# scroll-tech/zkvm-prover

Measured on AMD Instinct MI355X. Metric: chunk STARK proofs/sec (2^22-row trace), higher is better.
Workload: dtype u32; 1 GPU; full STARK proof: 2^22 x 300 degree-3 AIR + 2^22 x 2 Fibonacci AIR, blow-up 2, 100 queries, PoW 16+16 (SURVEY.md 8(d) cfg #4); proof_bytes=1128348, resident_key_bytes_per_pipeline=13503716096, inflight_per_gpu=3, parallelism=3 independent proof(s) in flight per GPU (one HIP stream each)

## Files before the change

include/zkhip.h:

```cpp
#ifndef ZKHIP_H
#define ZKHIP_H
#include <stddef.h>
#include <stdint.h>

#ifdef __cplusplus
extern "C" {
#endif

#define ZKHIP_OK 0
#define ZKHIP_ERR_NO_DEVICE (-1)
#define ZKHIP_ERR_HIP (-2)
#define ZKHIP_ERR_INVALID (-3)
#define ZKHIP_ERR_NOMEM (-4)
#define ZKHIP_ERR_SMALL_BUFFER (-5)
#define ZKHIP_ERR_POW_FAILED (-6)
#define ZKHIP_ERR_VERIFY (-7)
#define ZKHIP_ERR_CONSTRAINT (-8)

#define ZKHIP_DIGEST_WORDS 8

typedef struct zkhip_ctx zkhip_ctx;

uint32_t zkhip_version(void);

// ... 541 lines not shown
int zkhip_recursion_witness(zkhip_recursion *r, const uint8_t *const *proofs, const size_t *proof_lens, const uint32_t *const *const *child_pvs,
                            size_t n_present, uint32_t *node_pvs_out);
int zkhip_recursion_witness_uniform(zkhip_recursion *r, const uint8_t *const *proofs, const size_t *proof_lens, const uint32_t *const *const *child_pvs,
                                    const uint32_t *child_prep_commits, const int *child_is_leaf, const uint32_t leaf_commit[8],
                                    const uint32_t internal_commit[8], size_t n_present, uint32_t *node_pvs_out);
int zkhip_recursion_witness_deferral(zkhip_recursion *r, const uint8_t *const *proofs, const size_t *proof_lens, const uint32_t *const *const *child_pvs,
                                     const uint32_t *child_aux, const uint32_t acc_start[8], size_t n_present, uint32_t *node_pvs_out);
size_t zkhip_recursion_n_aux(const zkhip_recursion *r);
int zkhip_recursion_wires(const zkhip_recursion *r, uint32_t *out, size_t cap_words, size_t *n_words);
int zkhip_recursion_tracegen(zkhip_ctx *ctx, zkhip_recursion *r, uint32_t *d_gate_trace, uint32_t *d_p2_trace, uint32_t *d_pv_trace);

typedef struct {
    int host_sponge;
    uint32_t host_sponge_min_words;
    int jit;
    uint32_t jit_min_log_work;
    char jit_cache_dir[256];
    int quot_slices;
    uint32_t grind_sweep_shift;
    uint32_t coop_max_log, coop_inj_max_log;
    uint32_t top_max_log;
    uint32_t commit_parts, side_cus;
    uint32_t witness_threads;
    int pin_witness, parallel_queries;
    int self_check;
    int tree_store_early;
    uint32_t hash_block;
    int coop_fused;
    int rows_in_bulk;
    uint32_t rows_coop_max_log;
    uint32_t ntt_log_lanes;
    uint32_t quot_streams;
    uint32_t ntt_pass_form;
} zkhip_config;
int zkhip_tables_canonical(zkhip_ctx *ctx, int on);
int zkhip_jit_prewarm(const zkhip_air *airs, size_t n_airs, unsigned log_blowup, const char *cache_dir, size_t *n_ok);
void zkhip_config_default(zkhip_config *out);
unsigned zkhip_host_cpus(void);
int zkhip_ctx_get_config(zkhip_ctx *ctx, zkhip_config *out);
int zkhip_has_test_kernels(void);
int zkhip_ctx_set_config(zkhip_ctx *ctx, const zkhip_config *cfg);
int zkhip_set_process_config(const zkhip_config *cfg);

int zkhip_profile_enable(zkhip_ctx *ctx, int on);
typedef struct {
    char name[48];
    uint64_t launches;
    double total_ms;
} zkhip_kernel_stat;
int zkhip_profile_read(zkhip_ctx *ctx, zkhip_kernel_stat *out, size_t cap);
int zkhip_profile_reset(zkhip_ctx *ctx);

#ifdef __cplusplus
}
#endif
#endif
```

integration/hip-backend/src/ffi.rs:

```rust
#![allow(non_camel_case_types)]
use std::os::raw::{c_char, c_double, c_int, c_uint, c_void};

pub const ZKHIP_OK: c_int = 0;
pub const ZKHIP_ERR_NO_DEVICE: c_int = -1;
pub const ZKHIP_ERR_HIP: c_int = -2;
pub const ZKHIP_ERR_INVALID: c_int = -3;
pub const ZKHIP_ERR_NOMEM: c_int = -4;
pub const ZKHIP_ERR_SMALL_BUFFER: c_int = -5;
pub const ZKHIP_ERR_POW_FAILED: c_int = -6;
pub const ZKHIP_ERR_VERIFY: c_int = -7;
pub const ZKHIP_ERR_CONSTRAINT: c_int = -8;
pub const ZKHIP_DIGEST_WORDS: usize = 8;
pub const ZKHIP_KECCAK_F_WIDTH: usize = 2633;
pub const ZKHIP_INT256_ALU_WIDTH: usize = 101;
pub const ZKHIP_INT256_MUL_WIDTH: usize = 161;
pub const ZKHIP_MODMUL_WIDTH: usize = 325;
pub const ZKHIP_EC_WIDTH: usize = 772;
pub const ZKHIP_FP2_WIDTH: usize = 648;
pub const ZKHIP_FP2_RECORD_WORDS: usize = 33;
pub const ZKHIP_INT256_CMP_WIDTH: usize = 103;
pub const ZKHIP_INT256_SHIFT_WIDTH: usize = 189;
pub const ZKHIP_EC_RECORD_WORDS: usize = 41;
pub const ZKHIP_GKR_MAX_LOG_N: c_uint = 28;
pub const ZKHIP_WHIR_MAX_ROUNDS: usize = 32;
// ... 173 lines not shown
    pub min_log_height: [c_uint; 2],
    pub n_leaf_shapes: usize,
    pub app_id: *const u32,
    pub region_index: u32,
}

#[repr(C)]
#[derive(Clone, Copy)]
pub struct zkhip_config {
    pub host_sponge: c_int,
    pub host_sponge_min_words: u32,
    pub jit: c_int,
    pub jit_min_log_work: u32,
    pub jit_cache_dir: [c_char; 256],
    pub quot_slices: c_int,
    pub grind_sweep_shift: u32,
    pub coop_max_log: u32,
    pub coop_inj_max_log: u32,
    pub top_max_log: u32,
    pub commit_parts: u32,
    pub side_cus: u32,
    pub witness_threads: u32,
    pub pin_witness: c_int,
    pub parallel_queries: c_int,
    pub self_check: c_int,
    pub tree_store_early: c_int,
    pub hash_block: u32,
    pub coop_fused: c_int,
    pub rows_in_bulk: c_int,
    pub rows_coop_max_log: u32,
    pub ntt_log_lanes: u32,
    pub quot_streams: u32,
    pub ntt_pass_form: u32,
}

#[repr(C)]
#[derive(Clone, Copy)]
pub struct zkhip_kernel_stat {
    pub name: [c_char; 48],
    pub launches: u64,
    pub total_ms: c_double,
}

extern "C" {
    pub fn zkhip_version() -> u32;

    pub fn zkhip_ctx_create(device: c_int, out: *mut *mut zkhip_ctx) -> c_int;
    pub fn zkhip_ctx_destroy(ctx: *mut zkhip_ctx);
    pub fn zkhip_last_error(ctx: *const zkhip_ctx) -> *const c_char;
    pub fn zkhip_set_stream(ctx: *mut zkhip_ctx, hip_stream: *mut c_void) -> c_int;
    pub fn zkhip_sync(ctx: *mut zkhip_ctx) -> c_int;
    pub fn zkhip_set_commit_pipeline(ctx: *mut zkhip_ctx, parts: c_uint) -> c_int;
    pub fn zkhip_set_cu_partition(ctx: *mut zkhip_ctx, side_cus: c_uint) -> c_int;

    pub fn zkhip_malloc(ctx: *mut zkhip_ctx, bytes: usize, dptr: *mut *mut c_void) -> c_int;
    pub fn zkhip_free(ctx: *mut zkhip_ctx, dptr: *mut c_void) -> c_int;
    pub fn zkhip_h2d(ctx: *mut zkhip_ctx, dst: *mut c_void, src: *const c_void, bytes: usize) -> c_int;
    pub fn zkhip_d2h(ctx: *mut zkhip_ctx, dst: *mut c_void, src: *const c_void, bytes: usize) -> c_int;
    pub fn zkhip_host_alloc(ctx: *mut zkhip_ctx, bytes: usize, hptr: *mut *mut c_void) -> c_int;
    pub fn zkhip_host_free(ctx: *mut zkhip_ctx, hptr: *mut c_void) -> c_int;
    pub fn zkhip_h2d_async(ctx: *mut zkhip_ctx, dst: *mut c_void, src_pinned: *const c_void, bytes: usize) -> c_int;
    pub fn zkhip_zero(ctx: *mut zkhip_ctx, dptr: *mut c_void, bytes: usize) -> c_int;
    pub fn zkhip_to_monty(ctx: *mut zkhip_ctx, d: *mut u32, n: usize) -> c_int;
    pub fn zkhip_from_monty(ctx: *mut zkhip_ctx, d: *mut u32, n: usize) -> c_int;

    pub fn zkhip_ntt_batch(ctx: *mut zkhip_ctx, d_mat: *mut u32, log_n: c_uint, width: usize, stride: usize,
// ... 381 lines not shown
```

zkvm-prover_amd/_binding.py:

```python
import ctypes as C
import os
import re

import numpy as np

P = 2013265921
_HERE = os.path.dirname(os.path.abspath(__file__))
_ROOT = os.path.dirname(_HERE)
_LIB = None


class ZkhipError(RuntimeError):
    pass


def library_path():
    return os.path.join(_HERE, "libzkhip.so")


def declared_symbols():
    with open(os.path.join(_ROOT, "include", "zkhip.h")) as f:
        txt = f.read()
    txt = re.sub(r"/\*.*?\*/", "", txt, flags=re.S)
    return sorted(set(re.findall(r"\b(zkhip_[a-z0-9_]+)\s*\(", txt)))
# ... 24 lines not shown
        return p


class _Air(C.Structure):
    _fields_ = [("program", C.POINTER(C.c_uint32)), ("program_len", C.c_size_t), ("log_height", C.c_uint),
                ("width", C.c_size_t), ("n_pvs", C.c_size_t), ("prep_trace", C.POINTER(C.c_uint32)),
                ("prep_commit", C.POINTER(C.c_uint32))]


class _ProofLayout(C.Structure):
    _fields_ = [(n, C.c_size_t) for n in ("n_words", "root_main", "roots_cached", "n_cached", "root_perm", "exposed", "n_exposed", "root_quot", "opened",
                                          "n_opened", "fri_layers", "n_fri_layers", "final_poly", "n_final_poly", "query_pow", "queries",
                                          "query_words", "n_queries")]


class _V1Summary(C.Structure):
    _fields_ = [(n, C.c_size_t) for n in ("n_proofs", "n_airs", "n_queries", "n_fri_layers", "n_final_poly", "n_main_commits",
                                          "n_after_challenge_commits", "n_preprocessed", "n_input_batches")] + \
               [("log_max_height", C.c_uint), ("log_blowup", C.c_uint), ("has_logup_pow", C.c_int), ("log_degree", C.c_uint * 64)]


class _RecursionStmt(C.Structure):
    _fields_ = [("n_state", C.c_size_t), ("start_air", C.POINTER(C.c_uint32)), ("start_idx", C.POINTER(C.c_uint32)),
                ("end_air", C.POINTER(C.c_uint32)), ("end_idx", C.POINTER(C.c_uint32)), ("child_is_node", C.c_int),
                ("uniform", C.c_int), ("min_log_height", C.c_uint * 2), ("n_leaf_shapes", C.c_size_t), ("app_id", C.POINTER(C.c_uint32)),
                ("region_index", C.c_uint32)]


class Config(C.Structure):
    _fields_ = [("host_sponge", C.c_int), ("host_sponge_min_words", C.c_uint32), ("jit", C.c_int), ("jit_min_log_work", C.c_uint32),
                ("jit_cache_dir", C.c_char * 256), ("quot_slices", C.c_int), ("grind_sweep_shift", C.c_uint32), ("coop_max_log", C.c_uint32),
                ("coop_inj_max_log", C.c_uint32), ("top_max_log", C.c_uint32), ("commit_parts", C.c_uint32), ("side_cus", C.c_uint32), ("witness_threads", C.c_uint32),
                ("pin_witness", C.c_int), ("parallel_queries", C.c_int), ("self_check", C.c_int), ("tree_store_early", C.c_int), ("hash_block", C.c_uint32), ("coop_fused", C.c_int),
                ("rows_in_bulk", C.c_int), ("rows_coop_max_log", C.c_uint32), ("ntt_log_lanes", C.c_uint32), ("quot_streams", C.c_uint32), ("ntt_pass_form", C.c_uint32)]

    @classmethod
    def default(cls):
        c = cls()
        load_library().zkhip_config_default(C.byref(c))
        return c


class _KernelStat(C.Structure):
    _fields_ = [("name", C.c_char * 48), ("launches", C.c_uint64), ("total_ms", C.c_double)]


def load_library():
    global _LIB
    if _LIB is not None:
        return _LIB
    path = library_path()
    if not os.path.exists(path):
        raise ZkhipError("libzkhip.so not built: run `python -c 'import __graft_entry__ as g; g.build()'` "
                         "(or make -C zkvm-prover_amd/csrc)")
    import torch

    lib = C.CDLL(path)
    vp, sz, u32p, uip = C.c_void_p, C.c_size_t, C.POINTER(C.c_uint32), C.POINTER(C.c_uint)
    sig = {
        "zkhip_version": (C.c_uint32, []),
        "zkhip_ctx_create": (C.c_int, [C.c_int, C.POINTER(vp)]),
        "zkhip_ctx_destroy": (None, [vp]),
        "zkhip_last_error": (C.c_char_p, [vp]),
        "zkhip_set_stream": (C.c_int, [vp, vp]),
        "zkhip_sync": (C.c_int, [vp]),
        "zkhip_set_commit_pipeline": (C.c_int, [vp, C.c_uint]),
        "zkhip_set_cu_partition": (C.c_int, [vp, C.c_uint]),
# ... 2017 lines not shown
```

zkvm-prover_amd/csrc/api.hip:

```cpp
#include <sched.h>
#include <cstring>
#include <thread>
#include <dlfcn.h>
#include <sys/stat.h>
#include <mutex>
#include <string.h>

#include <algorithm>
#include <mutex>
#include <unordered_map>

#include "transcript.hpp"
#include "zkhip_internal.hpp"

namespace zk {

int set_error(zkhip_ctx* ctx, int code, const std::string& msg) {
    if (ctx) ctx->last_error = msg;
    return code;
}

int get_scratch(zkhip_ctx* ctx, int slot, size_t bytes, void** out) {
    if (bytes == 0) bytes = 16;
    if (ctx->scratch_bytes[slot] < bytes) {
// ... 163 lines not shown
    }();
    return cached;
}

void zkhip_config_default(zkhip_config* c) {
    if (!c) return;
    auto num = [](const char* name, uint32_t dflt, uint32_t lo = 0, uint32_t hi = 0xffffffffu) {
        if (!getenv(name)) return dflt;
        const long long v = atoll(getenv(name));
        return (uint32_t)std::min<long long>(hi, std::max<long long>(lo, v));
    };
    memset(c, 0, sizeof *c);
    c->host_sponge = getenv("ZKHIP_NO_HOST_SPONGE") ? 0 : 1;
    c->host_sponge_min_words = num("ZKHIP_HOST_SPONGE_MIN_WORDS", 8192u);
    c->jit = getenv("ZKHIP_NO_JIT") ? 0 : getenv("ZKHIP_FORCE_JIT") ? 2 : 1;
    c->jit_min_log_work = num("ZKHIP_JIT_MIN_LOG_WORK", 26u, 0, 62);
    c->quot_slices = getenv("ZKHIP_NO_QUOT_SLICES") ? 0 : 1;
    c->grind_sweep_shift = num("ZKHIP_GRIND_SWEEP_SHIFT", 0u, 0, 8);
    c->coop_max_log = num("ZKHIP_COOP_MAX_LOG", 15u, 0, 27), c->coop_inj_max_log = num("ZKHIP_COOP_INJ_MAX_LOG", 15u, 0, 27);
    c->top_max_log = num("ZKHIP_TOP_MAX_LOG", 6u, 0, 8);
    c->commit_parts = num("ZKHIP_COMMIT_PARTS", 0u, 0, 8), c->side_cus = num("ZKHIP_SIDE_CUS", 0u);
    c->witness_threads = num("ZKHIP_WITNESS_THREADS", 0u);
    c->pin_witness = getenv("ZKHIP_NO_PIN_WITNESS") ? 0 : 1;
    c->parallel_queries = getenv("ZKHIP_RECURSION_SERIAL_QUERIES") ? 0 : 1;
    c->self_check = getenv("ZKHIP_SELF_CHECK") ? 1 : 0;
#ifdef ZKHIP_TEST_KERNELS
    c->tree_store_early = getenv("ZKHIP_TREE_STORE_EARLY") ? 1 : 0;
#endif
    c->hash_block = num("ZKHIP_HASH_BLOCK", 256u, 64, 768) / 64 * 64;
    c->coop_fused = getenv("ZKHIP_NO_COOP_FUSED") ? 0 : 1;
    c->rows_in_bulk = getenv("ZKHIP_NO_ROWS_IN_BULK") ? 0 : 1;
    c->rows_coop_max_log = num("ZKHIP_ROWS_COOP_MAX_LOG", 15u, 0, 27);
    c->ntt_log_lanes = num("ZKHIP_NTT_LOG_LANES", 10u, 8, 10);
    c->ntt_pass_form = num("ZKHIP_NTT_PASS_FORM", 0u, 0, 2);
    c->quot_streams = num("ZKHIP_QUOT_STREAMS", 0u, 0, 4);
    std::string dir;
    if (const char* e = getenv("ZKHIP_JIT_CACHE_DIR")) {
        dir = e;
    } else {
        Dl_info info;
        if (dladdr((const void*)&zkhip_config_default, &info) && info.dli_fname) {
            std::string p = info.dli_fname;
            const size_t slash = p.rfind('/');
            p = (slash == std::string::npos ? std::string(".") : p.substr(0, slash)) + "/jit_cache";
            struct stat st;
            if (stat(p.c_str(), &st) == 0 && S_ISDIR(st.st_mode)) dir = p;
        }
    }
    if (dir.size() < sizeof c->jit_cache_dir) memcpy(c->jit_cache_dir, dir.c_str(), dir.size() + 1);
}
extern "C++" {
namespace zk {
static zkhip_config g_process_config;
static std::once_flag g_process_config_once;
static std::mutex g_process_config_mu;
zkhip_config process_config() {
    std::call_once(g_process_config_once, [] { zkhip_config_default(&g_process_config); });
    std::lock_guard<std::mutex> lk(g_process_config_mu);
    return g_process_config;
}
}
}
int zkhip_set_process_config(const zkhip_config* cfg) {
    if (!cfg) return ZKHIP_ERR_INVALID;
    (void)zk::process_config();
    std::lock_guard<std::mutex> lk(zk::g_process_config_mu);
    zk::g_process_config = *cfg;
    return ZKHIP_OK;
}
int zkhip_tables_canonical(zkhip_ctx* ctx, int on) {
    if (!ctx) return ZKHIP_ERR_INVALID;
    ctx->tables_canonical = on != 0;
    return ZKHIP_OK;
}

int zkhip_has_test_kernels(void) {
#ifdef ZKHIP_TEST_KERNELS
    return 1;
#else
    return 0;
#endif
}

int zkhip_ctx_get_config(zkhip_ctx* ctx, zkhip_config* out) {
    if (!ctx || !out) return ZKHIP_ERR_INVALID;
    *out = ctx->cfg;
    return ZKHIP_OK;
}
int zkhip_ctx_set_config(zkhip_ctx* ctx, const zkhip_config* cfg) {
    if (!ctx || !cfg) return ZKHIP_ERR_INVALID;
    if (cfg->jit < 0 || cfg->jit > 2 || cfg->coop_max_log > 27 || cfg->coop_inj_max_log > 27 || cfg->rows_coop_max_log > 27 || cfg->ntt_log_lanes < 8 || cfg->ntt_log_lanes > 10 || cfg->ntt_pass_form > 2 || cfg->quot_streams > 4 || cfg->jit_min_log_work > 62 || cfg->top_max_log > 8 || cfg->grind_sweep_shift > 8 ||
        cfg->commit_parts > 8 || cfg->side_cus >= (unsigned)ctx->cu_count || cfg->hash_block < 64 || cfg->hash_block > 768 || cfg->hash_block % 64)
        return set_error(ctx, ZKHIP_ERR_INVALID, "zkhip_ctx_set_config: field out of range (jit 0..2, coop_* <= 27, rows_coop_max_log <= 27, ntt_log_lanes 8..10, ntt_pass_form <= 2, quot_streams <= 4, jit_min_log_work <= 62, top_max_log <= 8, grind_sweep_shift <= 8, commit_parts <= 8, side_cus < CUs, hash_block a multiple of 64 in 64..768)");
#ifndef ZKHIP_TEST_KERNELS
    if (cfg->tree_store_early)
        return set_error(ctx, ZKHIP_ERR_INVALID, "zkhip_ctx_set_config: tree_store_early names TEST kernels that this library was built without (libzkhip_test.so holds them)");
#endif
    ZK_TRY(zkhip_set_cu_partition(ctx, cfg->side_cus));
    ctx->cfg = *cfg;
    ctx->cfg.jit_cache_dir[sizeof ctx->cfg.jit_cache_dir - 1] = 0;
    ctx->commit_parts = cfg->commit_parts;
    return ZKHIP_OK;
}

void zkhip_ctx_destroy(zkhip_ctx* ctx) {
    if (!ctx) return;
    (void)hipSetDevice(ctx->device);
    (void)hipStreamSynchronize(ctx->stream);
    profile_flush(ctx);
    if (ctx->d_tw_fwd) (void)hipFree(ctx->d_tw_fwd);
    if (ctx->d_tw_inv) (void)hipFree(ctx->d_tw_inv);
    for (auto& kv : ctx->lde_tables) (void)hipFree(kv.second);
    for (int i = 0; i < 8; i++)
        if (ctx->scratch[i]) (void)hipFree(ctx->scratch[i]);
    if (ctx->side_stream) (void)hipStreamDestroy(ctx->side_stream);
    if (ctx->hash_stream) (void)hipStreamDestroy(ctx->hash_stream);
    for (auto& q : ctx->quot_streams)
        if (q) (void)hipStreamDestroy(q);
    if (ctx->quot_fork) (void)hipEventDestroy(ctx->quot_fork);
    for (auto& e : ctx->quot_join)
        if (e) (void)hipEventDestroy(e);
    if (ctx->d_deferred_bad) (void)hipFree(ctx->d_deferred_bad);
    if (ctx->gkr_ws) (void)hipFree(ctx->gkr_ws);
    if (ctx->h_sponge) (void)hipHostFree(ctx->h_sponge);
    if (ctx->own_stream) (void)hipStreamDestroy(ctx->own_stream);
    for (auto& e : ctx->pipe_ev)
// ... 340 lines not shown
```

zkvm-prover_amd/csrc/ntt.hip:

```cpp
#include <stdlib.h>
#include <string.h>

#include <algorithm>

#include "lds_barrier.hpp"
#include "zkhip_internal.hpp"

namespace zk {

__global__ void k_gen_twiddles(uint32_t* fwd, uint32_t* inv, uint32_t w, uint32_t winv, size_t half) {
    size_t e = (size_t)blockIdx.x * blockDim.x + threadIdx.x;
    if (e >= half) return;
    fwd[e] = mpow(w, e);
    inv[e] = mpow(winv, e);
}

int ensure_twiddles(zkhip_ctx* ctx, unsigned log_n) {
    if (log_n < 1) log_n = 1;
    if (log_n > 27) return set_error(ctx, ZKHIP_ERR_INVALID, "transform size exceeds two-adicity 27");
    if (ctx->tw_log >= log_n) return ZKHIP_OK;
    unsigned want = std::max(log_n, 16u);
    if (ctx->d_tw_fwd) {
        ZK_HIP_CHECK(ctx, hipStreamSynchronize(ctx->stream));
        ZK_HIP_CHECK(ctx, hipFree(ctx->d_tw_fwd));
// ... 82 lines not shown
    }
    if (wide) {
        for (unsigned e = tid; e < total; e += nt) {
            unsigned r = e >> a.log_c, c = e & C_mask;
            dst[base + ((size_t)r << log_S) + c] = lds[e];
        }
    } else {
        const unsigned grp_mask = (1u << (a.log_r + log_S)) - 1u;
        for (unsigned e = tid; e < total; e += nt) {
            unsigned g = e >> (a.log_r + log_S), rem = e & grp_mask;
            unsigned r = rem >> log_S, low = rem & S_mask;
            dst[base + e] = lds[(r << a.log_c) + (g << log_S) + low];
        }
    }
}

struct Pass4Args {
    const uint32_t* src;
    uint32_t* dst;
    size_t src_col_stride, dst_col_stride;
    const uint32_t* tw;
    size_t in_x_stride, in_rs;
    size_t out_x_stride, out_hi_stride, out_lo_stride;
    unsigned log_sub, log_m, log_r, log_f, log_lo, tw_log, log_c;
    int in_tw;
    unsigned log_prev, log_tt;
    uint32_t tw_a, tw_bx;
    int br_src;
    const uint32_t* scale_col;
    const uint32_t* scale_row;
    const uint32_t* scale_rho;
    const uint32_t* const* src_cols;
    uint32_t* const* dst_cols;
};

template <int Q>
__device__ __forceinline__ void dif_unit(uint32_t (&v)[16], const uint32_t* twl, unsigned j, unsigned log_rq,
                                         unsigned tshift) {
#pragma unroll
    for (int t = 0; t < Q; t++) {
        constexpr int dummy = 0;
        (void)dummy;
        const int half = 1 << (Q - 1 - t);
#pragma unroll
        for (int kl = 0; kl < half; kl++) {
            const uint32_t w = twl[((j + ((unsigned)kl << log_rq)) << t) << tshift];
#pragma unroll
            for (int blk = 0; blk < (1 << t); blk++) {
                const int ka = blk * 2 * half + kl, kb = ka + half;
                const uint32_t x = v[ka], y = v[kb];
                v[ka] = madd(x, y);
                v[kb] = canon_signed(smml((int32_t)(x - y), (int32_t)w));
            }
        }
    }
}

template <int Q>
__device__ __forceinline__ void lds_round(uint32_t* lv, const uint32_t* twl, unsigned log_r, unsigned log_rcur,
                                          unsigned log_c, unsigned tid, unsigned nt) {
    const unsigned log_rq = log_rcur - Q;
    const unsigned n_units = 1u << (log_r - Q + log_c);
    const unsigned cmask = (1u << log_c) - 1u, pitch = (1u << log_c) + 1u;
    for (unsigned u = tid; u < n_units; u += nt) {
        const unsigned c = u & cmask, jj = u >> log_c;
        const unsigned j = jj & ((1u << log_rq) - 1u), blk = jj >> log_rq;
// ... 326 lines not shown
        t = mmul(sc, sr);
    } else {
        if constexpr (MODE == P4_IN_TW) {
            const uint32_t kc = bitrev32(F0 + c, LOG_F);
            const unsigned sh = a.tw_log - LOG_M;
            t = a.tw[(size_t)(kc * j) << sh];
            rho = a.tw[(size_t)(kc << LOG_RQ) << sh];
        }
        const global_words tile_src = uniform_global((a.src_cols ? a.src_cols[mcol] : a.src + mcol * a.src_col_stride) + ((size_t)sub << LOG_M) + F0);
        const uint32_t lane_off = (j << LOG_F) + c;
#pragma unroll
        for (int k = 0; k < 16; k++) v[k] = uniform_global(tile_src + ((size_t)k << (LOG_RQ + LOG_F)))[lane_off];
    }
#pragma unroll
    for (unsigned i = 0; i < (R >> 1) / NT; i++) twl[tid + i * NT] = twe[i];
    if constexpr (MODE != P4_PLAIN) scale_geometric(v, t, rho);
    zk_syncthreads();
    {
        uint32_t w[15];
        load_unit_twiddles<4, LOG_RQ, 0>(twl, j, w);
        dif_unit_w<4>(v, w);
        uint32_t* base = lv + j * pitch + c;
#pragma unroll
        for (int k = 0; k < 16; k++) base[(k << LOG_RQ) * pitch] = v[k];
    }
    zk_syncthreads();
    lds_rounds_ct<LOG_R, LOG_C, LOG_RQ, NT>(lv, twl, tid);
    const global_words dst = uniform_global((a.dst_cols ? a.dst_cols[mcol] : a.dst + mcol * a.dst_col_stride) + ((size_t)sub << LOG_M) + ((size_t)F0 << LOG_R));
    const uint32_t* lrow = lv + tid * pitch;
#pragma unroll
    for (unsigned i = 0; i < (R * C) / NT; i++) {
        const unsigned cc = (NT * i) >> LOG_R, p0 = (NT * i) & (R - 1u);
        uniform_global(dst + ((size_t)cc << LOG_R) + p0)[tid] = lrow[p0 * pitch + cc];
    }
}

struct LdeFusedArgs {
    const uint32_t* src;
    size_t src_col_stride;
    uint32_t* dst;
    size_t dst_col_stride;
    const uint32_t *tw_inv, *tw_fwd;
    unsigned tw_log, log_m, log_cosets;
    const uint32_t *scale_col, *scale_row, *scale_rho;
};
template <int LOG_R, int LOG_C, int MIN_WAVES>
__global__ __launch_bounds__(1024, MIN_WAVES) void k_ntt_lde_fused(LdeFusedArgs a) {
    constexpr int LOG_T = 10;
    static_assert(LOG_R - 4 + LOG_C == LOG_T, "one radix-16 unit per lane");
    constexpr unsigned NT = 1u << LOG_T;
    extern __shared__ uint32_t sm[];
    constexpr unsigned R = 1u << LOG_R, C = 1u << LOG_C, pitch = C + 1u;
    constexpr int LOG_RQ = LOG_R - 4;
    constexpr unsigned log_f = LOG_R;
    uint32_t* lv = sm;
    uint32_t* twl = sm + R * pitch;
    const unsigned tid = threadIdx.x;
    for (unsigned e = tid; e < (R >> 1); e += NT) twl[e] = a.tw_inv[(size_t)e << (a.tw_log - LOG_R)];
    const size_t mcol = blockIdx.y;
    unsigned tile = blockIdx.x;
    if (LOG_C == 3) {
        unsigned k = gridDim.x >> 3;
        if (k > 16u) k = 16u;
        if (k >= 2u && (k & (k - 1u)) == 0 && (gridDim.x & (8u * k - 1u)) == 0) {
            const unsigned within = tile & (8u * k - 1u);
            tile = (tile & ~(8u * k - 1u)) | ((within & 7u) * k) | (within >> 3);
// ... 89 lines not shown
static constexpr unsigned MAX_LOG_R = 11;
static constexpr unsigned P4_MIN_LOG_M = 12;

struct BrSrc {
    const uint32_t *scale_col, *scale_row, *scale_rho;
};
static unsigned fourstep_split(unsigned log_n, unsigned a[3]) {
    const unsigned n_pass = std::max(2u, (log_n + MAX_LOG_R - 1) / MAX_LOG_R);
    a[0] = a[1] = a[2] = 0;
    for (unsigned p = 0; p < n_pass; p++) a[p] = log_n / n_pass + (p < log_n % n_pass ? 1 : 0);
    return n_pass;
}
static int pass_scratch(zkhip_ctx* ctx, unsigned log_n, size_t words, uint32_t** t1, uint32_t** t2) {
    const bool three = log_n > 2 * MAX_LOG_R;
    void* tmp;
    ZK_TRY(get_scratch(ctx, 4, words * 4 * (three ? 2 : 1), &tmp));
    *t1 = (uint32_t*)tmp;
    *t2 = three ? *t1 + words : nullptr;
    return ZKHIP_OK;
}

typedef void (*Pass4Kernel)(Pass4Args);
struct Pass4Shape {
    unsigned log_r, log_c, log_t;
    Pass4Kernel kernel;
};
#define ZK_P4_CT(R_, C_, T_) {R_, C_, T_, k_ntt_pass4_ct<R_, C_, T_>}
static const Pass4Shape P4_SHAPES[] = {
    ZK_P4_CT(11, 3, 10), ZK_P4_CT(10, 4, 10), ZK_P4_CT(9, 5, 10), ZK_P4_CT(8, 6, 10), ZK_P4_CT(7, 7, 10),
    ZK_P4_CT(10, 3, 9),  ZK_P4_CT(9, 4, 9),   ZK_P4_CT(8, 5, 9),  ZK_P4_CT(7, 6, 9),
    ZK_P4_CT(10, 2, 8),  ZK_P4_CT(9, 3, 8),   ZK_P4_CT(8, 4, 8),  ZK_P4_CT(7, 5, 8),
};
#undef ZK_P4_CT
static const Pass4Kernel P4_SQ11[3] = {k_ntt_pass4_ct_sq<ShapeSq11, P4_PLAIN>, k_ntt_pass4_ct_sq<ShapeSq11, P4_IN_TW>,
                                       k_ntt_pass4_ct_sq<ShapeSq11, P4_BR_SRC>};
static bool pass4_is_sq11(const Pass4Args& pa, unsigned n_pass, unsigned n_x, unsigned log_n) {
    return n_pass == 2 && n_x == 1 && log_n == 22 && pa.log_r == 11 && pa.log_f == 11 && pa.log_c == 3 && pa.log_lo == 0 && pa.in_x_stride == 0 &&
           pa.out_x_stride == 0 && pa.out_hi_stride == ((size_t)1 << 11) && !(pa.br_src && pa.in_tw) &&
           (!pa.in_tw || (pa.log_prev == 11 && pa.log_tt == 22 && pa.tw_a == 1 && pa.tw_bx == 0));
}
static Pass4Kernel pass4_kernel_for(const Pass4Args& pa, unsigned log_t, int pass_form, unsigned n_pass, unsigned n_x, unsigned log_n) {
    if (pass_form == 0 && pass4_is_sq11(pa, n_pass, n_x, log_n)) return P4_SQ11[pa.br_src ? P4_BR_SRC : pa.in_tw ? P4_IN_TW : P4_PLAIN];
    for (const Pass4Shape& sh : P4_SHAPES)
        if (sh.log_r == pa.log_r && sh.log_c == pa.log_c && sh.log_t == log_t) return sh.kernel;
    return k_ntt_pass4;
}

static int ntt_dif_fourstep(zkhip_ctx* ctx, const uint32_t* src, size_t src_stride, uint32_t* dst, size_t dst_stride,
                            uint32_t* tmp, uint32_t* tmp2, size_t tmp_stride, unsigned log_n, size_t width,
                            unsigned log_sub, bool inverse, const BrSrc* brsrc = nullptr,
                            const uint32_t* const* src_cols = nullptr, uint32_t* const* dst_cols = nullptr) {
    static DeviceOnce attr_set;
    if (attr_set.need(ctx->device)) {
        const int lds_max = ((17u << MAX_LOG_R) + (1u << (MAX_LOG_R - 1))) * 4;
        for (const Pass4Shape& sh : P4_SHAPES) ZK_HIP_CHECK(ctx, hipFuncSetAttribute((const void*)sh.kernel, hipFuncAttributeMaxDynamicSharedMemorySize, lds_max));
        for (Pass4Kernel k : P4_SQ11) ZK_HIP_CHECK(ctx, hipFuncSetAttribute((const void*)k, hipFuncAttributeMaxDynamicSharedMemorySize, lds_max));
        ZK_HIP_CHECK(ctx, hipFuncSetAttribute((const void*)k_ntt_pass4, hipFuncAttributeMaxDynamicSharedMemorySize, lds_max));
        attr_set.mark(ctx->device);
    }
    unsigned a[3];
    const unsigned n_pass = fourstep_split(log_n, a);
    const uint32_t* tw = inverse ? ctx->d_tw_inv : ctx->d_tw_fwd;
    auto launch = [&](Pass4Args& pa, const uint32_t* s, size_t ss, uint32_t* d, size_t ds, unsigned n_x) -> int {
        pa.src = s;
        pa.src_col_stride = ss;
        pa.dst = d;
        pa.dst_col_stride = ds;
        pa.tw = tw;
        pa.tw_log = ctx->tw_log;
        pa.log_sub = log_sub;
        pa.log_m = log_n;
        const unsigned R = 1u << pa.log_r;
        pa.log_c = pa.log_r >= 11 ? 3u : (pa.log_r >= 7 ? 14u - pa.log_r : 4u);
        unsigned log_t = 10;
        if (pa.log_r >= 7 && pa.log_r <= 10 && ctx->cfg.ntt_log_lanes >= 8 && ctx->cfg.ntt_log_lanes <= 9) {
            const unsigned lc = ctx->cfg.ntt_log_lanes + 4 - pa.log_r;
            if (lc >= 2 && lc <= pa.log_f) log_t = ctx->cfg.ntt_log_lanes, pa.log_c = lc;
        }
        if (pa.log_c > pa.log_f) pa.log_c = pa.log_f;
        const unsigned C = 1u << pa.log_c;
        const unsigned threads = std::min(1024u, std::max(64u, (R >> 4) * C));
        const size_t lds = ((size_t)R * (C + 1) + (R >> 1)) * 4;
        dim3 grid(n_x << (pa.log_f - pa.log_c), (unsigned)(width << log_sub));
        KernelScope ks(ctx, inverse ? "ntt_pass_inv" : "ntt_pass_fwd");
        hipLaunchKernelGGL(pass4_kernel_for(pa, log_t, ctx->cfg.ntt_pass_form, n_pass, n_x, log_n), grid, dim3(threads), lds, ctx->stream, pa);
        ZK_HIP_CHECK(ctx, hipGetLastError());
        return ZKHIP_OK;
    };
    Pass4Args pa;
    memset(&pa, 0, sizeof pa);
    auto first_pass_src = [&]() {
        if (brsrc) {
            pa.br_src = 1;
            pa.scale_col = brsrc->scale_col, pa.scale_row = brsrc->scale_row, pa.scale_rho = brsrc->scale_rho;
        }
    };
    if (n_pass == 2) {
        const unsigned a1 = a[0], a2 = a[1];
        pa.log_r = a1, pa.log_f = a2, pa.in_x_stride = 0, pa.in_rs = (size_t)1 << a2;
        pa.out_x_stride = 0, pa.out_hi_stride = (size_t)1 << a1, pa.out_lo_stride = 0, pa.log_lo = 0, pa.in_tw = 0;
        first_pass_src();
        pa.src_cols = src_cols;
        ZK_TRY(launch(pa, src, src_stride, tmp, tmp_stride, 1));
        pa.src_cols = nullptr, pa.dst_cols = nullptr;
        pa.br_src = 0;
        pa.log_r = a2, pa.log_f = a1, pa.in_rs = (size_t)1 << a1, pa.out_hi_stride = (size_t)1 << a2;
        pa.in_tw = 1, pa.log_prev = a1, pa.log_tt = log_n, pa.tw_a = 1, pa.tw_bx = 0;
        pa.dst_cols = dst_cols;
        ZK_TRY(launch(pa, tmp, tmp_stride, dst, dst_stride, 1));
        pa.src_cols = nullptr, pa.dst_cols = nullptr;
    } else {
        const unsigned a1 = a[0], a2 = a[1], a3 = a[2];
        pa.log_r = a1, pa.log_f = a2 + a3, pa.in_x_stride = 0, pa.in_rs = (size_t)1 << (a2 + a3);
        pa.out_x_stride = 0, pa.log_lo = a3, pa.out_lo_stride = (size_t)1 << (a1 + a2), pa.out_hi_stride = (size_t)1 << a1;
        pa.in_tw = 0;
        first_pass_src();
        pa.src_cols = src_cols;
        ZK_TRY(launch(pa, src, src_stride, tmp, tmp_stride, 1));
// ... 459 lines not shown
```

Before: 13.83 proofs/s.

## Process runs of columns per block in square 2^11 NTT pass, prefetching next column

Adds a variant of the square 2^11x2^11 four-step NTT pass kernel in which each block handles a run of consecutive matrix columns (default 4). Twiddles are loaded into LDS once per block, and the global load of the next column is issued before the current column's results are written out, overlapping load latency with the LDS butterfly rounds and the stores. The variant becomes the default (pass_form 0), and the old kernel stays reachable as pass_form 3. In exchange the grid gets fewer blocks, which may reduce occupancy and tail balance, and register pressure rises from the prefetched values.

```diff
diff --git a/include/zkhip.h b/include/zkhip.h
--- a/include/zkhip.h
+++ b/include/zkhip.h
@@ -597,6 +597,7 @@
     uint32_t ntt_log_lanes;
     uint32_t quot_streams;
     uint32_t ntt_pass_form;
+    uint32_t ntt_col_run;
 } zkhip_config;
 int zkhip_tables_canonical(zkhip_ctx *ctx, int on);
 int zkhip_jit_prewarm(const zkhip_air *airs, size_t n_airs, unsigned log_blowup, const char *cache_dir, size_t *n_ok);
diff --git a/integration/hip-backend/src/ffi.rs b/integration/hip-backend/src/ffi.rs
--- a/integration/hip-backend/src/ffi.rs
+++ b/integration/hip-backend/src/ffi.rs
@@ -229,6 +229,7 @@
     pub ntt_log_lanes: u32,
     pub quot_streams: u32,
     pub ntt_pass_form: u32,
+    pub ntt_col_run: u32,
 }
 
 #[repr(C)]
diff --git a/zkvm-prover_amd/_binding.py b/zkvm-prover_amd/_binding.py
--- a/zkvm-prover_amd/_binding.py
+++ b/zkvm-prover_amd/_binding.py
@@ -80,7 +80,8 @@
                 ("jit_cache_dir", C.c_char * 256), ("quot_slices", C.c_int), ("grind_sweep_shift", C.c_uint32), ("coop_max_log", C.c_uint32),
                 ("coop_inj_max_log", C.c_uint32), ("top_max_log", C.c_uint32), ("commit_parts", C.c_uint32), ("side_cus", C.c_uint32), ("witness_threads", C.c_uint32),
                 ("pin_witness", C.c_int), ("parallel_queries", C.c_int), ("self_check", C.c_int), ("tree_store_early", C.c_int), ("hash_block", C.c_uint32), ("coop_fused", C.c_int),
-                ("rows_in_bulk", C.c_int), ("rows_coop_max_log", C.c_uint32), ("ntt_log_lanes", C.c_uint32), ("quot_streams", C.c_uint32), ("ntt_pass_form", C.c_uint32)]
+                ("rows_in_bulk", C.c_int), ("rows_coop_max_log", C.c_uint32), ("ntt_log_lanes", C.c_uint32), ("quot_streams", C.c_uint32), ("ntt_pass_form", C.c_uint32),
+                ("ntt_col_run", C.c_uint32)]
 
     @classmethod
     def default(cls):
diff --git a/zkvm-prover_amd/csrc/api.hip b/zkvm-prover_amd/csrc/api.hip
--- a/zkvm-prover_amd/csrc/api.hip
+++ b/zkvm-prover_amd/csrc/api.hip
@@ -219,7 +219,8 @@
     c->rows_in_bulk = getenv("ZKHIP_NO_ROWS_IN_BULK") ? 0 : 1;
     c->rows_coop_max_log = num("ZKHIP_ROWS_COOP_MAX_LOG", 15u, 0, 27);
     c->ntt_log_lanes = num("ZKHIP_NTT_LOG_LANES", 10u, 8, 10);
-    c->ntt_pass_form = num("ZKHIP_NTT_PASS_FORM", 0u, 0, 2);
+    c->ntt_pass_form = num("ZKHIP_NTT_PASS_FORM", 0u, 0, 3);
+    c->ntt_col_run = num("ZKHIP_NTT_COL_RUN", 4u, 1, 8);
     c->quot_streams = num("ZKHIP_QUOT_STREAMS", 0u, 0, 4);
     std::string dir;
     if (const char* e = getenv("ZKHIP_JIT_CACHE_DIR")) {
@@ -276,9 +277,9 @@
 }
 int zkhip_ctx_set_config(zkhip_ctx* ctx, const zkhip_config* cfg) {
     if (!ctx || !cfg) return ZKHIP_ERR_INVALID;
-    if (cfg->jit < 0 || cfg->jit > 2 || cfg->coop_max_log > 27 || cfg->coop_inj_max_log > 27 || cfg->rows_coop_max_log > 27 || cfg->ntt_log_lanes < 8 || cfg->ntt_log_lanes > 10 || cfg->ntt_pass_form > 2 || cfg->quot_streams > 4 || cfg->jit_min_log_work > 62 || cfg->top_max_log > 8 || cfg->grind_sweep_shift > 8 ||
+    if (cfg->jit < 0 || cfg->jit > 2 || cfg->coop_max_log > 27 || cfg->coop_inj_max_log > 27 || cfg->rows_coop_max_log > 27 || cfg->ntt_log_lanes < 8 || cfg->ntt_log_lanes > 10 || cfg->ntt_pass_form > 3 || cfg->ntt_col_run < 1 || cfg->ntt_col_run > 8 || cfg->quot_streams > 4 || cfg->jit_min_log_work > 62 || cfg->top_max_log > 8 || cfg->grind_sweep_shift > 8 ||
         cfg->commit_parts > 8 || cfg->side_cus >= (unsigned)ctx->cu_count || cfg->hash_block < 64 || cfg->hash_block > 768 || cfg->hash_block % 64)
-        return set_error(ctx, ZKHIP_ERR_INVALID, "zkhip_ctx_set_config: field out of range (jit 0..2, coop_* <= 27, rows_coop_max_log <= 27, ntt_log_lanes 8..10, ntt_pass_form <= 2, quot_streams <= 4, jit_min_log_work <= 62, top_max_log <= 8, grind_sweep_shift <= 8, commit_parts <= 8, side_cus < CUs, hash_block a multiple of 64 in 64..768)");
+        return set_error(ctx, ZKHIP_ERR_INVALID, "zkhip_ctx_set_config: field out of range (jit 0..2, coop_* <= 27, rows_coop_max_log <= 27, ntt_log_lanes 8..10, ntt_pass_form <= 3, ntt_col_run 1..8, quot_streams <= 4, jit_min_log_work <= 62, top_max_log <= 8, grind_sweep_shift <= 8, commit_parts <= 8, side_cus < CUs, hash_block a multiple of 64 in 64..768)");
 #ifndef ZKHIP_TEST_KERNELS
     if (cfg->tree_store_early)
         return set_error(ctx, ZKHIP_ERR_INVALID, "zkhip_ctx_set_config: tree_store_early names TEST kernels that this library was built without (libzkhip_test.so holds them)");
diff --git a/zkvm-prover_amd/csrc/ntt.hip b/zkvm-prover_amd/csrc/ntt.hip
--- a/zkvm-prover_amd/csrc/ntt.hip
+++ b/zkvm-prover_amd/csrc/ntt.hip
@@ -138,6 +138,7 @@
     const uint32_t* scale_rho;
     const uint32_t* const* src_cols;
     uint32_t* const* dst_cols;
+    unsigned n_mcols, col_run;
 };
 
 template <int Q>
@@ -530,6 +531,108 @@
     for (unsigned i = 0; i < (R * C) / NT; i++) {
         const unsigned cc = (NT * i) >> LOG_R, p0 = (NT * i) & (R - 1u);
         uniform_global(dst + ((size_t)cc << LOG_R) + p0)[tid] = lrow[p0 * pitch + cc];
+    }
+}
+
+__device__ __forceinline__ const uint32_t* column_pointer(const uint32_t* const* table, size_t i) {
+    typedef __attribute__((address_space(4))) const uint64_t* constant_words64;
+    return (const uint32_t*)((constant_words64)(uint64_t)table)[i];
+}
+template <class SH, int MODE>
+__global__ __launch_bounds__(1 << SH::LOG_T, 8) void k_ntt_pass4_ct_sq_run(Pass4Args a) {
+    constexpr int LOG_R = SH::LOG_R, LOG_C = SH::LOG_C, LOG_T = SH::LOG_T;
+    constexpr int LOG_F = LOG_R, LOG_M = 2 * LOG_R, LOG_RQ = LOG_R - 4;
+    constexpr unsigned NT = 1u << LOG_T, R = 1u << LOG_R, C = 1u << LOG_C, pitch = C + 1u;
+    static_assert(LOG_C == 3 && LOG_RQ + LOG_C == LOG_T && LOG_R >= LOG_T && (R >> 1) % NT == 0 && LOG_F - LOG_C >= 7, "[2^11 x 8] tiles of 1024 lanes");
+    extern __shared__ uint32_t sm[];
+    const unsigned tid = threadIdx.x;
+    const unsigned sub = blockIdx.y & ((1u << a.log_sub) - 1u);
+    const unsigned mcol0 = (blockIdx.y >> a.log_sub) * a.col_run;
+    const unsigned n_run = min(a.col_run, a.n_mcols - mcol0);
+    unsigned tile = blockIdx.x;
+    tile = (tile & ~127u) | ((tile & 7u) << 4) | ((tile & 127u) >> 3);
+    const unsigned F0 = tile << LOG_C;
+    const unsigned c = tid & (C - 1u), jj = tid >> LOG_C;
+    const unsigned j = ((jj & 3u) << 3) | ((jj >> 2) & 7u) | (jj & ~31u);
+    uint32_t twe[(R >> 1) / NT];
+#pragma unroll
+    for (unsigned i = 0; i < (R >> 1) / NT; i++) twe[i] = a.tw[(size_t)(tid + i * NT) << (a.tw_log - LOG_R)];
+    uint32_t t = 0, rho = 0, sc = 0, sr = 0, v[16];
+    if constexpr (MODE == P4_BR_SRC) {
+        sc = a.scale_col[((size_t)sub << LOG_F) + F0 + c], sr = a.scale_row[((size_t)sub << LOG_RQ) + j];
+        rho = a.scale_rho[sub];
+    } else if constexpr (MODE == P4_IN_TW) {
+        const uint32_t kc = bitrev32(F0 + c, LOG_F);
+        const unsigned sh = a.tw_log - LOG_M;
+        t = a.tw[(size_t)(kc * j) << sh];
+        rho = a.tw[(size_t)(kc << LOG_RQ) << sh];
+    }
+    auto load_column = [&](size_t mcol, unsigned lane) {
+        const unsigned cl = lane & (C - 1u), jq = lane >> LOG_C;
+        const unsigned jl = ((jq & 3u) << 3) | ((jq >> 2) & 7u) | (jq & ~31u);
+        if constexpr (MODE == P4_BR_SRC) {
+            typedef uint32_t words4 __attribute__((ext_vector_type(4)));
+            typedef __attribute__((address_space(1))) const words4* global_quads;
+            const uint32_t src_off = (bitrev32(F0 + cl, LOG_F) << LOG_R) + (bitrev32(jl, LOG_RQ) << 4);
+            const global_quads ch = (global_quads)(uniform_global(a.src + mcol * a.src_col_stride) + src_off);
+            const words4 q0 = ch[0], q1 = ch[1], q2 = ch[2], q3 = ch[3];
+            const uint32_t wv[16] = {q0.x, q0.y, q0.z, q0.w, q1.x, q1.y, q1.z, q1.w, q2.x, q2.y, q2.z, q2.w, q3.x, q3.y, q3.z, q3.w};
+#pragma unroll
+            for (int k = 0; k < 16; k++) v[k] = wv[((k & 1) << 3) | ((k & 2) << 1) | ((k & 4) >> 1) | ((k & 8) >> 3)];
+        } else {
+            const global_words tile_src = uniform_global((a.src_cols ? column_pointer(a.src_cols, mcol) : a.src + mcol * a.src_col_stride) + ((size_t)sub << LOG_M) + F0);
+            const uint32_t src_off = (jl << LOG_F) + cl;
+#pragma unroll
+            for (int k = 0; k < 16; k++) v[k] = uniform_global(tile_src + ((size_t)k << (LOG_RQ + LOG_F)))[src_off];
+        }
+    };
+    load_column(mcol0, tid);
+#pragma unroll
+    for (unsigned i = 0; i < (R >> 1) / NT; i++) sm[R * pitch + tid + i * NT] = twe[i];
+    if constexpr (MODE == P4_BR_SRC) t = mmul(sc, sr);
+#pragma unroll
+    for (int k = 0; k < 16; k++) asm volatile("" : "+v"(v[k]));
+    asm volatile("" : "+v"(t), "+v"(rho));
+    for (unsigned q = 0; q < n_run; q++) {
+        const size_t mcol = (size_t)mcol0 + q;
+        if constexpr (MODE != P4_PLAIN) {
+            uint32_t tq = t, rq = rho;
+            asm volatile("" : "+v"(tq), "+v"(rq));
+            scale_geometric(v, tq, rq);
+        }
+        zk_syncthreads();
+        unsigned tl = tid;
+        asm volatile("" : "+v"(tl));
+        tl &= NT - 1u;
+        unsigned zero = 0;
+        asm volatile("" : "+s"(zero));
+        uint32_t* const lv = sm + zero;
+        uint32_t* const twl = lv + R * pitch;
+        {
+            const unsigned cl = tl & (C - 1u), jq = tl >> LOG_C;
+            const unsigned jl = ((jq & 3u) << 3) | ((jq >> 2) & 7u) | (jq & ~31u);
+            uint32_t w[15];
+            load_unit_twiddles<4, LOG_RQ, 0>(twl, jl, w);
+            dif_unit_w<4>(v, w);
+            uint32_t* base = lv + jl * pitch + cl;
+#pragma unroll
+            for (int k = 0; k < 16; k++) base[(k << LOG_RQ) * pitch] = v[k];
+        }
+        zk_syncthreads();
+        lds_rounds_ct<LOG_R, LOG_C, LOG_RQ, NT>(lv, twl, tl);
+        const bool more = q + 1 < n_run;
+        if (more) load_column(mcol + 1, tl);
+        const global_words dst = uniform_global((a.dst_cols ? column_pointer((const uint32_t* const*)a.dst_cols, mcol) : a.dst + mcol * a.dst_col_stride) + ((size_t)sub << LOG_M) + ((size_t)F0 << LOG_R));
+        const uint32_t* lrow = lv + tl * pitch;
+#pragma unroll
+        for (unsigned i = 0; i < (R * C) / NT; i++) {
+            const unsigned cc = (NT * i) >> LOG_R, p0 = (NT * i) & (R - 1u);
+            uniform_global(dst + ((size_t)cc << LOG_R) + p0)[tl] = lrow[p0 * pitch + cc];
+        }
+        if (more) {
+#pragma unroll
+            for (int k = 0; k < 16; k++) asm volatile("" : "+v"(v[k]));
+        }
     }
 }
 
@@ -685,6 +788,8 @@
     ZK_P4_CT(10, 2, 8),  ZK_P4_CT(9, 3, 8),   ZK_P4_CT(8, 4, 8),  ZK_P4_CT(7, 5, 8),
 };
 #undef ZK_P4_CT
+static const Pass4Kernel P4_SQ11_RUN[3] = {k_ntt_pass4_ct_sq_run<ShapeSq11, P4_PLAIN>, k_ntt_pass4_ct_sq_run<ShapeSq11, P4_IN_TW>,
+                                           k_ntt_pass4_ct_sq_run<ShapeSq11, P4_BR_SRC>};
 static const Pass4Kernel P4_SQ11[3] = {k_ntt_pass4_ct_sq<ShapeSq11, P4_PLAIN>, k_ntt_pass4_ct_sq<ShapeSq11, P4_IN_TW>,
                                        k_ntt_pass4_ct_sq<ShapeSq11, P4_BR_SRC>};
 static bool pass4_is_sq11(const Pass4Args& pa, unsigned n_pass, unsigned n_x, unsigned log_n) {
@@ -693,7 +798,8 @@
            (!pa.in_tw || (pa.log_prev == 11 && pa.log_tt == 22 && pa.tw_a == 1 && pa.tw_bx == 0));
 }
 static Pass4Kernel pass4_kernel_for(const Pass4Args& pa, unsigned log_t, int pass_form, unsigned n_pass, unsigned n_x, unsigned log_n) {
-    if (pass_form == 0 && pass4_is_sq11(pa, n_pass, n_x, log_n)) return P4_SQ11[pa.br_src ? P4_BR_SRC : pa.in_tw ? P4_IN_TW : P4_PLAIN];
+    if ((pass_form == 0 || pass_form == 3) && pass4_is_sq11(pa, n_pass, n_x, log_n))
+        return (pass_form == 0 ? P4_SQ11_RUN : P4_SQ11)[pa.br_src ? P4_BR_SRC : pa.in_tw ? P4_IN_TW : P4_PLAIN];
     for (const Pass4Shape& sh : P4_SHAPES)
         if (sh.log_r == pa.log_r && sh.log_c == pa.log_c && sh.log_t == log_t) return sh.kernel;
     return k_ntt_pass4;
@@ -708,6 +814,7 @@
         const int lds_max = ((17u << MAX_LOG_R) + (1u << (MAX_LOG_R - 1))) * 4;
         for (const Pass4Shape& sh : P4_SHAPES) ZK_HIP_CHECK(ctx, hipFuncSetAttribute((const void*)sh.kernel, hipFuncAttributeMaxDynamicSharedMemorySize, lds_max));
         for (Pass4Kernel k : P4_SQ11) ZK_HIP_CHECK(ctx, hipFuncSetAttribute((const void*)k, hipFuncAttributeMaxDynamicSharedMemorySize, lds_max));
+        for (Pass4Kernel k : P4_SQ11_RUN) ZK_HIP_CHECK(ctx, hipFuncSetAttribute((const void*)k, hipFuncAttributeMaxDynamicSharedMemorySize, lds_max));
         ZK_HIP_CHECK(ctx, hipFuncSetAttribute((const void*)k_ntt_pass4, hipFuncAttributeMaxDynamicSharedMemorySize, lds_max));
         attr_set.mark(ctx->device);
     }
@@ -735,8 +842,14 @@
         const unsigned threads = std::min(1024u, std::max(64u, (R >> 4) * C));
         const size_t lds = ((size_t)R * (C + 1) + (R >> 1)) * 4;
         dim3 grid(n_x << (pa.log_f - pa.log_c), (unsigned)(width << log_sub));
+        const Pass4Kernel kernel = pass4_kernel_for(pa, log_t, ctx->cfg.ntt_pass_form, n_pass, n_x, log_n);
+        pa.n_mcols = (unsigned)width, pa.col_run = 1;
+        if (std::find(std::begin(P4_SQ11_RUN), std::end(P4_SQ11_RUN), kernel) != std::end(P4_SQ11_RUN)) {
+            pa.col_run = ctx->cfg.ntt_col_run;
+            grid.y = (unsigned)(((width + pa.col_run - 1) / pa.col_run) << log_sub);
+        }
         KernelScope ks(ctx, inverse ? "ntt_pass_inv" : "ntt_pass_fwd");
-        hipLaunchKernelGGL(pass4_kernel_for(pa, log_t, ctx->cfg.ntt_pass_form, n_pass, n_x, log_n), grid, dim3(threads), lds, ctx->stream, pa);
+        hipLaunchKernelGGL(kernel, grid, dim3(threads), lds, ctx->stream, pa);
         ZK_HIP_CHECK(ctx, hipGetLastError());
         return ZKHIP_OK;
     };
```

Result: no change. 13.96 proofs/s, median of 6 (+0.9%).
